# antonilo/unsupervised_detection

Measured on AMD Instinct MI355X. Metric: frame-pairs/sec per adversarial step, DAVIS 480p batch4, 1/2/4/8 GPU, higher is better.
Workload: dtype f32

## Files before the change

unsupervised_detection_amd/csrc/elementwise.h:

```cpp
#pragma once
#include "common.h"
namespace udet {
int launch_resize_bilinear_fwd(const float* x, int ldx, int x_coff, int N, int H, int W, float* y, int ldy, int y_coff,
                               int OH, int OW, int C, float mul, float div, hipStream_t s);
int launch_resize_bilinear_bwd(const float* dy, int ldy, int y_coff, int N, int OH, int OW, float* dx, int ldx, int x_coff,
                               int H, int W, int C, int accumulate, hipStream_t s);
int launch_upb_ring(const float* x, int ld, int N, int H, int W, float* xh, hipStream_t s);
int launch_upb_ring_fold(const float* dxh, int ld, int N, int H, int W, float* dx, hipStream_t s);
int launch_share_samples(float* buf, long P, int ld, int coff, int C, int copies, hipStream_t s);
int launch_fold_samples(float* buf, long P, int ld, int coff, int C, int copies, hipStream_t s);
int launch_emit_du(const float* d, const float* a, float* u, long P, int ld, int coff, int C, int act, float alpha, hipStream_t s);
int launch_pool2x2_sum(const float* du, float* dx, int N, int H, int W, int C, hipStream_t s);
int launch_pack_pwc_input(const float* i1, const float* i2, float* x8, long P, hipStream_t s);
int launch_gen_input(const float* img, const float* f, double* part, float* gin, int B, long HW, hipStream_t s);
size_t flow_stats_doubles(int B);
int launch_mask_rec_inputs(const float* logits, const float* f, float* mask, float* fin, long P, int ncalls, hipStream_t s);
int launch_pack_imgin(const float* img, float* imgin, long P, int ncalls, hipStream_t s);
int launch_losses(const float* f, const float* mask, const float* pred, long HW, int B, float cbn, float eps,
                  float num_pixels, float* part, float* losses, float* coef, float* sums, hipStream_t s);
size_t loss_part_floats(int B);
int launch_rec_loss_bwd(const float* f, const float* mask, const float* pred, float* dpred, long BHW, float cbn,
                        float inv_np, hipStream_t s);
int launch_gen_loss_bwd(const float* f, const float* mask, const float* pred, const float* coef, float* dpred,
                        float* dmask, long HW, int B, float cbn, hipStream_t s);
int launch_mask_bwd(const float* dmask, const float* dfin, const float* f, const float* mask, float* dlogits, long P,
                    hipStream_t s);
int launch_grad_absmean(const float* g, const long* seg_off, const long* seg_len, int nvars, float* vmean, float thresh,
                        float* out, hipStream_t s);
int launch_adam(float* w, float* g, float* m, float* v, long n, float lr_t, float b1, float b2, float eps, float clip,
                const float* flag, uint64_t seed, uint64_t step, hipStream_t s, int mode = 0, const int* skip = nullptr);
int launch_nonfinite_count(const float* g, long n, int* out, hipStream_t s);
int launch_flow_normalize(const float* f, double* part, float* out, int B, long HW, hipStream_t s);
int launch_charbonnier(const float* gt, const float* pred, const float* mask, int mc, int B, long HW, float cbn, float* part,
                       float* out, hipStream_t s);
int launch_crop_flip_resize(const void* src, int src_u8, int nearest, int N, int H, int W, int C, const int* prm, float* dst, int OH,
                            int OW, float div, float add, hipStream_t s);
int launch_crop_flip_resize_ragged(const void* src, int src_u8, int nearest, int N, int C, const long long* offsets, const int* hw,
                                   const int* prm, float* dst, int OH, int OW, float div, float add, hipStream_t s);
int launch_mask_stats(const float* pred, const float* gt, int N, int H, int W, float threshold, float gt_threshold, double* out,
                      hipStream_t s);
int launch_boundary_stats(const float* pred, const float* gt, const double* stats8, int N, int H, int W, float threshold,
                          float gt_threshold, int radius, unsigned long long* counts4, unsigned char* bmap_pred,
                          unsigned char* bmap_gt, hipStream_t s);
size_t restore_workspace_bytes(int n);
int launch_restore_masks_ragged(const float* masks, int n, int mh, int mw, const long long* offsets, const int* tab, const int* coef,
                                int max_h, int max_w, unsigned char* out, int* amax, unsigned char* binary, double threshold,
                                void* workspace, hipStream_t s);
size_t components_workspace_bytes(size_t total_pixels, int n);
int launch_select_components_ragged(const unsigned char* binary, const unsigned char* gt, int n, const long long* offsets, const int* hw,
                                    int max_h, int max_w, size_t total_pixels, int connectivity, int mode, int* labels,
                                    unsigned char* selected, long long* info, void* workspace, hipStream_t s);
size_t component_boxes_workspace_bytes(size_t total_pixels, int n);
int launch_component_boxes_ragged(const int* labels, const unsigned char* score, int n, const long long* offsets, const int* hw, int max_h,
                                  int max_w, size_t total_pixels, int min_area, int k, long long* dets, long long* counts, void* workspace,
                                  hipStream_t s);
int launch_draw_boxes_ragged(unsigned char* rgb, int n, const long long* offsets, const int* hw, const long long* dets,
                             const long long* counts, int k, int thickness, unsigned colour, hipStream_t s);
int launch_fill_uniform(float* x, long n, uint64_t seed, float lo, float hi, hipStream_t s);
int launch_axpy(const float* x, float* y, long n, float a, int accumulate, hipStream_t s);
}
```

unsupervised_detection_amd/csrc/elementwise.hip:

```cpp
#include "common.h"
#include "elementwise.h"

namespace udet {

static inline int grid_for(long total, int cap = 4096) {
  long nb = (total + 255) / 256;
  if (nb > cap) nb = cap;
  if (nb < 1) nb = 1;
  return (int)nb;
}

template <typename T>
__device__ __forceinline__ T wave_sum(T v) {
#pragma unroll
  for (int o = 32; o > 0; o >>= 1) v += __shfl_down(v, o, 64);
  return v;
}
template <typename T>
__device__ __forceinline__ T block_sum(T v, T* sm ) {
  v = wave_sum(v);
  __syncthreads();
  if ((threadIdx.x & 63) == 0) sm[threadIdx.x >> 6] = v;
  __syncthreads();
  return sm[0] + sm[1] + sm[2] + sm[3];
// ... 252 lines not shown
                       C / 4, accumulate);
    UDET_HIP(hipGetLastError());
    return UDET_OK;
  }
  const long total = (long)N * H * W * C;
  hipLaunchKernelGGL(resize_bilinear_bwd_kernel, dim3(grid_for(total)), dim3(256), 0, s, dy, ldy, y_coff, N, OH, OW, dx,
                     ldx, x_coff, H, W, C, accumulate);
  UDET_HIP(hipGetLastError());
  return UDET_OK;
}

__global__ __launch_bounds__(256) void pool2x2_sum_kernel(const float* __restrict__ du, float* __restrict__ dx, int N, int H,
                                                          int W, int C) {
  const int c4n = C >> 2;
  const long total = (long)N * H * W * c4n;
  for (long e = (long)blockIdx.x * 256 + threadIdx.x; e < total; e += (long)gridDim.x * 256) {
    const int c4 = (int)(e % c4n);
    const long pix = e / c4n;
    const int x = (int)(pix % W), y = (int)((pix / W) % H), n = (int)(pix / ((long)W * H));
    const float* b = du + ((((long)n * 2 * H + 2 * y) * 2 * W) + 2 * x) * C + c4 * 4;
    const float4 a0 = *reinterpret_cast<const float4*>(b), a1 = *reinterpret_cast<const float4*>(b + C);
    const float4 a2 = *reinterpret_cast<const float4*>(b + (long)2 * W * C), a3 = *reinterpret_cast<const float4*>(b + (long)2 * W * C + C);
    float4 o;
    o.x = (a0.x + a1.x) + (a2.x + a3.x);
    o.y = (a0.y + a1.y) + (a2.y + a3.y);
    o.z = (a0.z + a1.z) + (a2.z + a3.z);
    o.w = (a0.w + a1.w) + (a2.w + a3.w);
    *reinterpret_cast<float4*>(dx + pix * C + c4 * 4) = o;
  }
}
int launch_pool2x2_sum(const float* du, float* dx, int N, int H, int W, int C, hipStream_t s) {
  hipLaunchKernelGGL(pool2x2_sum_kernel, dim3(grid_for((long)N * H * W * (C / 4))), dim3(256), 0, s, du, dx, N, H, W, C);
  UDET_HIP(hipGetLastError());
  return UDET_OK;
}

__global__ __launch_bounds__(256) void emit_du_kernel(const float* __restrict__ d, const float* __restrict__ a,
                                                      float* __restrict__ u, long P, int ld, int coff, int C, int act,
                                                      float alpha) {
  const long total = P * C;
  for (long e = (long)blockIdx.x * 256 + threadIdx.x; e < total; e += (long)gridDim.x * 256) {
    const long pix = e / C;
    const long o = pix * ld + coff + (e - pix * C);
    u[o] = d[o] * act_dfo(a[o], act, alpha);
  }
}
int launch_emit_du(const float* d, const float* a, float* u, long P, int ld, int coff, int C, int act, float alpha, hipStream_t s) {
  hipLaunchKernelGGL(emit_du_kernel, dim3(grid_for(P * C)), dim3(256), 0, s, d, a, u, P, ld, coff, C, act, alpha);
  UDET_HIP(hipGetLastError());
  return UDET_OK;
}

template <int V, bool FOLD>
__global__ __launch_bounds__(256) void share_fold_kernel(float* __restrict__ buf, long P, int ld, int coff, int C, int copies) {
  const int CV = C / V;
  const long total = P * CV;
  for (long e = (long)blockIdx.x * 256 + threadIdx.x; e < total; e += (long)gridDim.x * 256) {
    const long pix = e / CV;
    const long o = pix * ld + coff + (e - pix * CV) * V;
    if (V == 4) {
      float4 v = *reinterpret_cast<const float4*>(buf + o);
      for (int k = 1; k < copies; ++k) {
        float4* q = reinterpret_cast<float4*>(buf + o + (long)k * P * ld);
        if (FOLD) {
          const float4 w = *q;
          v.x += w.x; v.y += w.y; v.z += w.z; v.w += w.w;
        } else {
          *q = v;
        }
      }
      if (FOLD) *reinterpret_cast<float4*>(buf + o) = v;
    } else {
      float v = buf[o];
      for (int k = 1; k < copies; ++k) {
        if (FOLD) v += buf[o + (long)k * P * ld];
        else buf[o + (long)k * P * ld] = v;
      }
      if (FOLD) buf[o] = v;
    }
  }
}
static int launch_share_fold(float* buf, long P, int ld, int coff, int C, int copies, bool fold, hipStream_t s) {
  if (copies < 2 || C < 1) return UDET_OK;
  const bool v4 = (ld % 4 == 0) && (coff % 4 == 0) && (C % 4 == 0);
  const long n = P * (v4 ? C / 4 : C);
  if (v4) {
    if (fold) hipLaunchKernelGGL((share_fold_kernel<4, true>), dim3(grid_for(n)), dim3(256), 0, s, buf, P, ld, coff, C, copies);
    else hipLaunchKernelGGL((share_fold_kernel<4, false>), dim3(grid_for(n)), dim3(256), 0, s, buf, P, ld, coff, C, copies);
  } else {
    if (fold) hipLaunchKernelGGL((share_fold_kernel<1, true>), dim3(grid_for(n)), dim3(256), 0, s, buf, P, ld, coff, C, copies);
    else hipLaunchKernelGGL((share_fold_kernel<1, false>), dim3(grid_for(n)), dim3(256), 0, s, buf, P, ld, coff, C, copies);
  }
  UDET_HIP(hipGetLastError());
  return UDET_OK;
}
int launch_share_samples(float* buf, long P, int ld, int coff, int C, int copies, hipStream_t s) {
  return launch_share_fold(buf, P, ld, coff, C, copies, false, s);
}
int launch_fold_samples(float* buf, long P, int ld, int coff, int C, int copies, hipStream_t s) {
  return launch_share_fold(buf, P, ld, coff, C, copies, true, s);
}

__global__ __launch_bounds__(256) void pack_pwc_input_kernel(const float* __restrict__ i1, const float* __restrict__ i2,
                                                             float* __restrict__ x8, long P) {
  for (long e = (long)blockIdx.x * 256 + threadIdx.x; e < 2 * P; e += (long)gridDim.x * 256) {
    const float* s = e < P ? i1 + e * 3 : i2 + (e - P) * 3;
    float4 a = make_float4(s[0] + 0.5f, s[1] + 0.5f, s[2] + 0.5f, 0.f);
    *reinterpret_cast<float4*>(x8 + e * 4) = a;
  }
}
int launch_pack_pwc_input(const float* i1, const float* i2, float* x8, long P, hipStream_t s) {
  hipLaunchKernelGGL(pack_pwc_input_kernel, dim3(grid_for(2 * P)), dim3(256), 0, s, i1, i2, x8, P);
  UDET_HIP(hipGetLastError());
  return UDET_OK;
}

#define FS_BLOCKS 32
__global__ __launch_bounds__(256) void flow_stats_kernel(const float* __restrict__ f, long HW, double* __restrict__ part) {
  __shared__ double sm[4];
  const int n = blockIdx.y;
  double s0 = 0, s1 = 0, q0 = 0, q1 = 0;
  for (long p = (long)blockIdx.x * 256 + threadIdx.x; p < HW; p += (long)gridDim.x * 256) {
    const float2 v = *reinterpret_cast<const float2*>(f + ((long)n * HW + p) * 2);
    s0 += v.x; s1 += v.y;
    q0 += (double)v.x * v.x; q1 += (double)v.y * v.y;
  }
  s0 = block_sum(s0, sm); s1 = block_sum(s1, sm); q0 = block_sum(q0, sm); q1 = block_sum(q1, sm);
  if (threadIdx.x == 0) {
    double* o = part + ((long)n * FS_BLOCKS + blockIdx.x) * 4;
    o[0] = s0; o[1] = s1; o[2] = q0; o[3] = q1;
  }
}
__global__ __launch_bounds__(256) void pack_gen_input_kernel(const float* __restrict__ img, const float* __restrict__ f,
                                                             const double* __restrict__ part, float* __restrict__ gin,
                                                             long HW) {
  __shared__ float st[4];
  const int n = blockIdx.y;
  if (threadIdx.x < 2) {
    double s = 0, q = 0;
    for (int b = 0; b < FS_BLOCKS; ++b) {
      s += part[((long)n * FS_BLOCKS + b) * 4 + threadIdx.x];
      q += part[((long)n * FS_BLOCKS + b) * 4 + 2 + threadIdx.x];
    }
    const double mean = s / (double)HW, var = q / (double)HW - mean * mean;
    st[threadIdx.x] = (float)mean;
    st[2 + threadIdx.x] = sqrtf((float)var);
  }
  __syncthreads();
  const float m0 = st[0], m1 = st[1], d0 = st[2], d1 = st[3];
  for (long p = (long)blockIdx.x * 256 + threadIdx.x; p < HW; p += (long)gridDim.x * 256) {
    const long q = (long)n * HW + p;
    const float2 v = *reinterpret_cast<const float2*>(f + q * 2);
    *reinterpret_cast<float4*>(gin + q * 8) = make_float4(img[q * 3], img[q * 3 + 1], img[q * 3 + 2], (v.x - m0) / d0);
// ... 60 lines not shown
  }
}
int launch_mask_rec_inputs(const float* logits, const float* f, float* mask, float* fin, long P, int ncalls, hipStream_t s) {
  hipLaunchKernelGGL(mask_rec_inputs_kernel, dim3(grid_for(P)), dim3(256), 0, s, logits, f, mask, fin, P, ncalls);
  UDET_HIP(hipGetLastError());
  return UDET_OK;
}
__global__ __launch_bounds__(256) void pack_imgin_kernel(const float* __restrict__ img, float* __restrict__ imgin, long P,
                                                         int ncalls) {
  for (long q = (long)blockIdx.x * 256 + threadIdx.x; q < P; q += (long)gridDim.x * 256) {
    const float4 im = make_float4(img[q * 3], img[q * 3 + 1], img[q * 3 + 2], 0.f);
    for (int k = 0; k < ncalls; ++k) *reinterpret_cast<float4*>(imgin + (k * P + q) * 4) = im;
  }
}
int launch_pack_imgin(const float* img, float* imgin, long P, int ncalls, hipStream_t s) {
  hipLaunchKernelGGL(pack_imgin_kernel, dim3(grid_for(P)), dim3(256), 0, s, img, imgin, P, ncalls);
  UDET_HIP(hipGetLastError());
  return UDET_OK;
}

__device__ __forceinline__ float charb(float e, float cbn) {
  const float s = e * e + 0.001f * 0.001f;
  return cbn == 0.5f ? sqrtf(s) : powf(s, cbn);
}
__device__ __forceinline__ float charb_d(float e, float cbn) {
  const float s = e * e + 0.001f * 0.001f;
  return cbn == 0.5f ? e / sqrtf(s) : cbn * powf(s, cbn - 1.f) * 2.f * e;
}
#define LS_BLOCKS 64
__global__ __launch_bounds__(256) void loss_sums_kernel(const float* __restrict__ f, const float* __restrict__ mask,
                                                        const float* __restrict__ pred , long HW, int B,
                                                        float cbn, float* __restrict__ part ) {
  __shared__ float sm[4];
  const int n = blockIdx.y;
  float R = 0, Rc = 0, Pp = 0, Dr = 0, Dc = 0;
  for (long p = (long)blockIdx.x * 256 + threadIdx.x; p < HW; p += (long)gridDim.x * 256) {
    const long q = (long)n * HW + p;
    const float2 fl = *reinterpret_cast<const float2*>(f + q * 2);
    const float2 a = *reinterpret_cast<const float2*>(pred + q * 2);
    const float2 b = *reinterpret_cast<const float2*>(pred + ((long)B * HW + q) * 2);
    const float2 c = *reinterpret_cast<const float2*>(pred + ((long)2 * B * HW + q) * 2);
    const float m = mask[q], cm = 1.f - m;
    const float pa = charb(fl.x - a.x, cbn) + charb(fl.y - a.y, cbn);
    const float pb = charb(fl.x - b.x, cbn) + charb(fl.y - b.y, cbn);
    const float pc = charb(fl.x - c.x, cbn) + charb(fl.y - c.y, cbn);
    R += pa * m; Rc += pb * cm; Pp += pc; Dr += pc * m; Dc += pc * cm;
  }
  R = block_sum(R, sm); Rc = block_sum(Rc, sm); Pp = block_sum(Pp, sm); Dr = block_sum(Dr, sm); Dc = block_sum(Dc, sm);
  if (threadIdx.x == 0) {
    float* o = part + ((long)n * LS_BLOCKS + blockIdx.x) * 5;
    o[0] = R; o[1] = Rc; o[2] = Pp; o[3] = Dr; o[4] = Dc;
  }
}
__global__ void loss_finish_kernel(const float* __restrict__ part, int B, float eps, float num_pixels,
                                   float* __restrict__ losses, float* __restrict__ coef, float* __restrict__ sums) {
  if (threadIdx.x != 0 || blockIdx.x != 0) return;
  float red = 0.f, redc = 0.f, rs = 0.f;
  for (int b = 0; b < B; ++b) {
    float v[5] = {0, 0, 0, 0, 0};
    for (int k = 0; k < LS_BLOCKS; ++k)
      for (int j = 0; j < 5; ++j) v[j] += part[((long)b * LS_BLOCKS + k) * 5 + j];
    const float D = v[3] + eps, Dc = v[4] + eps;
    red += 1.f - v[0] / D;
    redc += 1.f - v[1] / Dc;
    rs += v[0] + v[1] + v[2];
    coef[b * 4 + 0] = -1.f / (B * D);
    coef[b * 4 + 1] = v[0] / (B * D * D);
    coef[b * 4 + 2] = -1.f / (B * Dc);
    coef[b * 4 + 3] = v[1] / (B * Dc * Dc);
    for (int j = 0; j < 5; ++j) sums[b * 5 + j] = v[j];
    if (b == 0) { losses[4] = v[0]; losses[5] = v[1]; losses[6] = D; losses[7] = Dc; }
  }
  red /= B; redc /= B;
  losses[0] = red + redc;
  losses[1] = rs / num_pixels;
  losses[2] = red;
  losses[3] = redc;
}
int launch_losses(const float* f, const float* mask, const float* pred, long HW, int B, float cbn, float eps,
                  float num_pixels, float* part, float* losses, float* coef, float* sums, hipStream_t s) {
  hipLaunchKernelGGL(loss_sums_kernel, dim3(LS_BLOCKS, B), dim3(256), 0, s, f, mask, pred, HW, B, cbn, part);
  hipLaunchKernelGGL(loss_finish_kernel, dim3(1), dim3(64), 0, s, part, B, eps, num_pixels, losses, coef, sums);
  UDET_HIP(hipGetLastError());
  return UDET_OK;
}
size_t loss_part_floats(int B) { return (size_t)B * LS_BLOCKS * 5; }

__global__ __launch_bounds__(256) void charbonnier_sum_kernel(const float* __restrict__ gt, const float* __restrict__ pred,
                                                              const float* __restrict__ mask, int mc, long HW, float cbn,
                                                              float* __restrict__ part ) {
  __shared__ float sm[4];
  const int n = blockIdx.y;
  float acc = 0.f;
  for (long p = (long)blockIdx.x * 256 + threadIdx.x; p < HW; p += (long)gridDim.x * 256) {
    const long q = (long)n * HW + p;
    const float2 a = *reinterpret_cast<const float2*>(gt + q * 2);
    const float2 b = *reinterpret_cast<const float2*>(pred + q * 2);
    const float m0 = mask ? mask[q * mc] : 1.f, m1 = mask ? mask[q * mc + (mc - 1)] : 1.f;
    acc += charb(a.x - b.x, cbn) * m0 + charb(a.y - b.y, cbn) * m1;
  }
  acc = block_sum(acc, sm);
  if (threadIdx.x == 0) part[(long)n * LS_BLOCKS + blockIdx.x] = acc;
}
__global__ void charbonnier_finish_kernel(const float* __restrict__ part, int B, float* __restrict__ out) {
  const int b = blockIdx.x * blockDim.x + threadIdx.x;
  if (b >= B) return;
  float v = 0.f;
  for (int k = 0; k < LS_BLOCKS; ++k) v += part[(long)b * LS_BLOCKS + k];
  out[b] = v;
}
int launch_charbonnier(const float* gt, const float* pred, const float* mask, int mc, int B, long HW, float cbn, float* part,
                       float* out, hipStream_t s) {
  hipLaunchKernelGGL(charbonnier_sum_kernel, dim3(LS_BLOCKS, B), dim3(256), 0, s, gt, pred, mask, mc, HW, cbn, part);
  hipLaunchKernelGGL(charbonnier_finish_kernel, dim3((B + 63) / 64), dim3(64), 0, s, part, B, out);
  UDET_HIP(hipGetLastError());
  return UDET_OK;
}

__global__ __launch_bounds__(256) void rec_loss_bwd_kernel(const float* __restrict__ f, const float* __restrict__ mask,
                                                           const float* __restrict__ pred, float* __restrict__ dpred,
                                                           long BHW, float cbn, float inv_np) {
  for (long q = (long)blockIdx.x * 256 + threadIdx.x; q < BHW; q += (long)gridDim.x * 256) {
    const float2 fl = *reinterpret_cast<const float2*>(f + q * 2);
    const float m = mask[q], cm = 1.f - m;
    const float2 a = *reinterpret_cast<const float2*>(pred + q * 2);
    const float2 b = *reinterpret_cast<const float2*>(pred + (BHW + q) * 2);
    const float2 c = *reinterpret_cast<const float2*>(pred + (2 * BHW + q) * 2);
    *reinterpret_cast<float2*>(dpred + q * 2) = make_float2(-charb_d(fl.x - a.x, cbn) * m * inv_np, -charb_d(fl.y - a.y, cbn) * m * inv_np);
    *reinterpret_cast<float2*>(dpred + (BHW + q) * 2) = make_float2(-charb_d(fl.x - b.x, cbn) * cm * inv_np, -charb_d(fl.y - b.y, cbn) * cm * inv_np);
    *reinterpret_cast<float2*>(dpred + (2 * BHW + q) * 2) = make_float2(-charb_d(fl.x - c.x, cbn) * inv_np, -charb_d(fl.y - c.y, cbn) * inv_np);
  }
}
int launch_rec_loss_bwd(const float* f, const float* mask, const float* pred, float* dpred, long BHW, float cbn,
                        float inv_np, hipStream_t s) {
  hipLaunchKernelGGL(rec_loss_bwd_kernel, dim3(grid_for(BHW)), dim3(256), 0, s, f, mask, pred, dpred, BHW, cbn, inv_np);
// ... 11 lines not shown
    const float cR = coef[n * 4], cD = coef[n * 4 + 1], cRc = coef[n * 4 + 2], cDc = coef[n * 4 + 3];
    const float2 fl = *reinterpret_cast<const float2*>(f + q * 2);
    const float m = mask[q], cm = 1.f - m;
    const float2 a = *reinterpret_cast<const float2*>(pred + q * 2);
    const float2 b = *reinterpret_cast<const float2*>(pred + (BHW + q) * 2);
    const float2 c = *reinterpret_cast<const float2*>(pred + (2 * BHW + q) * 2);
    *reinterpret_cast<float2*>(dpred + q * 2) = make_float2(-cR * charb_d(fl.x - a.x, cbn) * m, -cR * charb_d(fl.y - a.y, cbn) * m);
    *reinterpret_cast<float2*>(dpred + (BHW + q) * 2) = make_float2(-cRc * charb_d(fl.x - b.x, cbn) * cm, -cRc * charb_d(fl.y - b.y, cbn) * cm);
    const float pa = charb(fl.x - a.x, cbn) + charb(fl.y - a.y, cbn);
    const float pb = charb(fl.x - b.x, cbn) + charb(fl.y - b.y, cbn);
    const float pc = charb(fl.x - c.x, cbn) + charb(fl.y - c.y, cbn);
    dmask[q] = cR * pa + cD * pc - cRc * pb - cDc * pc;
  }
}
int launch_gen_loss_bwd(const float* f, const float* mask, const float* pred, const float* coef, float* dpred,
                        float* dmask, long HW, int B, float cbn, hipStream_t s) {
  hipLaunchKernelGGL(gen_loss_bwd_kernel, dim3(grid_for((long)B * HW)), dim3(256), 0, s, f, mask, pred, coef, dpred, dmask,
                     HW, B, cbn);
  UDET_HIP(hipGetLastError());
  return UDET_OK;
}

__global__ __launch_bounds__(256) void mask_bwd_kernel(const float* __restrict__ dmask, const float* __restrict__ dfin,
                                                       const float* __restrict__ f, const float* __restrict__ mask,
                                                       float* __restrict__ dlogits , long P) {
  for (long q = (long)blockIdx.x * 256 + threadIdx.x; q < P; q += (long)gridDim.x * 256) {
    const float4 g0 = *reinterpret_cast<const float4*>(dfin + q * 4);
    const float4 g1 = *reinterpret_cast<const float4*>(dfin + (P + q) * 4);
    const float2 fl = *reinterpret_cast<const float2*>(f + q * 2);
    float dm = dmask[q];
    dm -= g0.x * fl.x + g0.y * fl.y + g0.w;
    dm += g1.x * fl.x + g1.y * fl.y + g1.w;
    const float m = mask[q];
    const float d0 = dm * m * (1.f - m) / 10.f;
    dlogits[q * 8] = d0;
    dlogits[q * 8 + 1] = -d0;
  }
}
int launch_mask_bwd(const float* dmask, const float* dfin, const float* f, const float* mask, float* dlogits, long P,
                    hipStream_t s) {
  hipLaunchKernelGGL(mask_bwd_kernel, dim3(grid_for(P)), dim3(256), 0, s, dmask, dfin, f, mask, dlogits, P);
  UDET_HIP(hipGetLastError());
  return UDET_OK;
}

#define GA_SPLIT 8
__global__ __launch_bounds__(256) void grad_absmean_kernel(const float* __restrict__ g, const long* __restrict__ seg_off,
                                                           const long* __restrict__ seg_len, float* __restrict__ vpart) {
  __shared__ float sm[4];
  const long off = seg_off[blockIdx.x], len = seg_len[blockIdx.x];
  const long b = len * blockIdx.y / GA_SPLIT, e = len * (blockIdx.y + 1) / GA_SPLIT;
  float s0 = 0.f, s1 = 0.f, s2 = 0.f, s3 = 0.f;
  long i = b + threadIdx.x;
  for (; i + 768 < e; i += 1024) {
    s0 += fabsf(g[off + i]);
    s1 += fabsf(g[off + i + 256]);
    s2 += fabsf(g[off + i + 512]);
    s3 += fabsf(g[off + i + 768]);
  }
  for (; i < e; i += 256) s0 += fabsf(g[off + i]);
  const float s = block_sum((s0 + s1) + (s2 + s3), sm);
  if (threadIdx.x == 0) vpart[blockIdx.x * GA_SPLIT + blockIdx.y] = s;
}
__global__ void grad_flag_kernel(const float* __restrict__ vpart, const long* __restrict__ seg_len, int nvars, float thresh,
                                 float* __restrict__ out ) {
  if (threadIdx.x == 0 && blockIdx.x == 0) {
    float s = 0.f;
    for (int i = 0; i < nvars; ++i) {
      float v = 0.f;
      for (int j = 0; j < GA_SPLIT; ++j) v += vpart[i * GA_SPLIT + j];
      s += v / (float)seg_len[i];
    }
    s /= (float)nvars;
    out[0] = s;
    out[1] = s < thresh ? 1.f : 0.f;
  }
}
int launch_grad_absmean(const float* g, const long* seg_off, const long* seg_len, int nvars, float* vmean, float thresh,
                        float* out, hipStream_t s) {
  hipLaunchKernelGGL(grad_absmean_kernel, dim3(nvars, GA_SPLIT), dim3(256), 0, s, g, seg_off, seg_len, vmean);
  hipLaunchKernelGGL(grad_flag_kernel, dim3(1), dim3(64), 0, s, vmean, seg_len, nvars, thresh, out);
  UDET_HIP(hipGetLastError());
  return UDET_OK;
}

__device__ __host__ __forceinline__ float udet_uniform01(uint64_t seed, uint64_t step, uint64_t idx) {
  uint64_t z = seed * 0x9E3779B97F4A7C15ull + step * 0xBF58476D1CE4E5B9ull + idx + 0x94D049BB133111EBull;
  z = (z ^ (z >> 30)) * 0xBF58476D1CE4E5B9ull;
  z = (z ^ (z >> 27)) * 0x94D049BB133111EBull;
  z = z ^ (z >> 31);
  return (float)(z >> 40) * (1.0f / 16777216.0f);
}

__global__ __launch_bounds__(256) void adam_kernel(float* __restrict__ w, float* __restrict__ g, float* __restrict__ m,
                                                   float* __restrict__ v, long n, float lr_t, float b1, float b2, float eps,
                                                   float clip, const float* __restrict__ flag, uint64_t seed,
                                                   uint64_t step, int mode, const int* __restrict__ skip) {
  if (skip && *skip != 0) return;
  const bool noise = flag && flag[1] != 0.f;
  for (long i = (long)blockIdx.x * 256 + threadIdx.x; i < n; i += (long)gridDim.x * 256) {
    float gi = g[i];
    if (mode != 2) {
      if (noise) gi = fabsf((udet_uniform01(seed, step, (uint64_t)i) * 2.f - 1.f) * clip);
      else gi = fminf(fmaxf(gi, -clip), clip);
      g[i] = gi;
      if (mode == 1) continue;
    }
    const float mi = m[i] + (gi - m[i]) * (1.f - b1);
    const float vi = v[i] + (gi * gi - v[i]) * (1.f - b2);
    m[i] = mi;
    v[i] = vi;
    w[i] = w[i] - lr_t * mi / (sqrtf(vi) + eps);
  }
}
__global__ __launch_bounds__(256) void fill_uniform_kernel(float* __restrict__ x, long n, uint64_t seed, float lo, float hi) {
  for (long i = (long)blockIdx.x * 256 + threadIdx.x; i < n; i += (long)gridDim.x * 256)
    x[i] = lo + (hi - lo) * udet_uniform01(seed, 0, (uint64_t)i);
}
int launch_fill_uniform(float* x, long n, uint64_t seed, float lo, float hi, hipStream_t s) {
  hipLaunchKernelGGL(fill_uniform_kernel, dim3(grid_for(n, 8192)), dim3(256), 0, s, x, n, seed, lo, hi);
  UDET_HIP(hipGetLastError());
  return UDET_OK;
}
__global__ __launch_bounds__(256) void mask_stats_kernel(const float* __restrict__ pred, const float* __restrict__ gt, int H, int W,
                                                         float threshold, float gt_threshold, double* __restrict__ out) {
  __shared__ double sm[4];
  const int n = blockIdx.x;
  const long HW = (long)H * W;
  double v[8] = {0, 0, 0, 0, 0, 0, 0, 0};
  for (long q = threadIdx.x; q < HW; q += 256) {
    const int y = (int)(q / W), x = (int)(q - (long)y * W);
    const float g = gt[n * HW + q];
    const bool pr = pred[n * HW + q] > threshold, gb = g > gt_threshold;
    const int strips = (y < 2) + (y >= H - 2) + (x < 2) + (x >= W - 2);
// ... 116 lines not shown
```

unsupervised_detection_amd/csrc/plan_step.hip:

```cpp
#include "conv_host.h"
#include "elementwise.h"
#include "plan_run.h"

namespace udet {

static const int PWC_CH[7] = {0, 16, 32, 64, 96, 128, 196};
static const char* const WARP_NAME[7] = {"", "", "warp_costvol2", "warp_costvol3", "warp_costvol4", "warp_costvol5", "warp_costvol6"};

static int pwc_forward_on(Plan* P, const float* img1, const float* img2, float* ws, const Lane& L0, const Lane& LH) {
  if (!P->pwc_packed) {
    set_error("pwc_forward: call udet_pack_pwc first");
    return UDET_ERR_ARG;
  }
  const Config& c = P->cfg;
  const Resolved& R = P->R;
  const int B = c.batch;
  hipStream_t s = L0.s;
  auto fwd = [&](int layer, int N, const Lane& ln) { return run_fwd(P, P->pwc[layer], N, ws, ln); };
  UDET_TRY(launch_pack_pwc_input(img1, img2, ws + P->buf(R.pwc_x8).off, (long)B * c.in_h * c.in_w, s));
  for (int l = 1; l <= 6; ++l)
    for (int j = 0; j < 3; ++j) UDET_TRY(fwd(R.pwc.pyr[l][j], 2 * B, L0));
  for (int l = 6; l >= 2; --l) {
    const int h = c.in_h >> l, w = c.in_w >> l, C = PWC_CH[l];
    const Buf& cb = P->buf(R.pwc_c[l]);
// ... 25 lines not shown
  if (P->prefetch_pending) (void)hipStreamWaitEvent(s, P->prefetch_ev, 0);
  return pwc_forward_on(P, img1, img2, ws, lane_of(P, s, 0), lane_of(P, s, 2));
}

static int plan_prepare_image(Plan* P, const float* img1, int dst, float* ws, hipStream_t s) {
  const Config& c = P->cfg;
  return launch_resize_bilinear_fwd(img1, 3, 0, c.batch, c.in_h, c.in_w, ws + P->buf(dst).off, 3, 0, c.img_h, c.img_w,
                                    3, 1.f, 1.f, s);
}
static int plan_prepare_flow(Plan* P, int dst, float* ws, hipStream_t s) {
  const Config& c = P->cfg;
  const Buf& ff = P->buf(P->R.flow_full);
  return launch_resize_bilinear_fwd(ws + ff.off, 2, 0, c.batch, c.in_h, c.in_w, ws + P->buf(dst).off, 2, 0, c.img_h,
                                    c.img_w, 2, 1.f, c.flow_normalizer, s);
}

int plan_prefetch(Plan* P, const float* img1, const float* img2, float* ws, hipStream_t s) {
  const Lane L0 = lane_of(P, s, 0), LC = lane_of(P, s, 4), LH = lane_of(P, s, 5);
  P->in_prefetch = true;
  P->ev_next_prefetch = 0;
  order_after(P, L0, LC);
  int rc = pwc_forward_on(P, img1, img2, ws, LC, LH);
  P->in_prefetch = false;
  UDET_TRY(rc);
  UDET_TRY(plan_prepare_flow(P, P->R.flow_next, ws, LC.s));
  UDET_TRY(plan_prepare_image(P, img1, P->R.image_next, ws, LC.s));
  if (!P->prefetch_ev) (void)hipEventCreateWithFlags(&P->prefetch_ev, hipEventDisableTiming);
  (void)hipEventRecord(P->prefetch_ev, LC.s);
  P->prefetch_pending = true;
  return UDET_OK;
}

int plan_generator_forward(Plan* P, float* ws, hipStream_t s) {
  const Config& c = P->cfg;
  const long HW = (long)c.img_h * c.img_w;
  const Lane L0 = lane_of(P, s, 0);
  double* part = reinterpret_cast<double*>(ws + P->small_off + 4096);
  UDET_TRY(launch_gen_input(ws + P->buf(P->R.image).off, ws + P->buf(P->R.flow).off, part, ws + P->buf(P->R.gen_in).off, c.batch, HW, s));
  for (const auto& L : P->gen) UDET_TRY(run_fwd(P, L, c.batch, ws, L0));
  return UDET_OK;
}
int plan_generator_layers(Plan* P, float* ws, hipStream_t s) {
  const Lane L0 = lane_of(P, s, 0);
  for (const auto& L : P->gen) UDET_TRY(run_fwd(P, L, P->cfg.batch, ws, L0));
  return UDET_OK;
}

static int rec_resize(Plan* P, int src, int dst, int N, float* ws, hipStream_t s) {
  const Buf &a = P->buf(src), &b = P->buf(dst);
  return launch_resize_bilinear_fwd(ws + a.off, a.ld, 0, N, a.h, a.w, ws + b.off, b.ld, 0, b.h, b.w, a.ld, 1.f, 1.f, s);
}
static int dec_src(const Resolved& R, int k) { return k == 5 ? R.rec_conv6 : R.rec_concat[k + 1]; }

static int share_enc_a_output(Plan* P, const Layer& L, int ncalls, float* ws, hipStream_t s) {
  const Buf& y = P->buf(L.y);
  if (ncalls > 1 && L.y_fanned_out) return launch_share_samples(ws + y.off, (long)P->cfg.batch * y.h * y.w, y.ld, L.y_coff, L.cout, ncalls, s);
  return UDET_OK;
}
static int plan_rec_image_branch(Plan* P, int ncalls, float* ws, const Lane& ln, bool with_layers = true) {
  const Config& c = P->cfg;
  if (ncalls < 1) return UDET_OK;
  const long Ppix = (long)c.batch * c.img_h * c.img_w;
  UDET_TRY(launch_pack_imgin(ws + P->buf(P->R.image).off, ws + P->buf(P->R.rec_imgin).off, Ppix, 1, ln.s));
  if (!with_layers) return UDET_OK;
  for (int i = 0; i < 9; ++i) {
    const Layer& L = P->rec[P->R.rec.enc[0][i]];
    UDET_TRY(run_fwd(P, L, c.batch, ws, ln));
    UDET_TRY(share_enc_a_output(P, L, ncalls, ws, ln.s));
  }
  P->enc_a_shared = true;
  return UDET_OK;
}

int plan_recover_forward(Plan* P, int ncalls, float* ws, hipStream_t s, bool inputs_prepacked, bool skip_enc_a, bool enc_a_input_packed) {
  const Config& c = P->cfg;
  const Resolved& R = P->R;
  const int B = c.batch, N = ncalls * B;
  const long Ppix = (long)B * c.img_h * c.img_w;
  const Lane L0 = lane_of(P, s, 0);
  if (!inputs_prepacked)
    UDET_TRY(launch_mask_rec_inputs(ws + P->buf(R.gen_a17).off, ws + P->buf(R.flow).off, ws + P->buf(R.mask).off, ws + P->buf(R.rec_fin).off,
                                    Ppix, ncalls, s));
  if (ncalls < 1) return UDET_OK;
  auto enc = [&](int e, int i) -> const Layer& { return P->rec[R.rec.enc[e][i]]; };
  if (!skip_enc_a && pairs_on(P)) {
    if (!inputs_prepacked && !enc_a_input_packed) UDET_TRY(plan_rec_image_branch(P, ncalls, ws, L0, false));
    for (int i = 0; i < 9; ++i) {
      const Layer& La = enc(0, i);
      UDET_TRY(run_fwd_pair(P, La, inputs_prepacked ? N : B, enc(1, i), N, ws, L0));
      if (!inputs_prepacked) UDET_TRY(share_enc_a_output(P, La, ncalls, ws, s));
    }
    P->enc_a_shared = !inputs_prepacked;
  } else {
    if (!skip_enc_a) {
      if (inputs_prepacked) {
        for (int i = 0; i < 9; ++i) UDET_TRY(run_fwd(P, enc(0, i), N, ws, L0));
        P->enc_a_shared = false;
      } else {
        UDET_TRY(plan_rec_image_branch(P, ncalls, ws, L0));
      }
    }
    for (int i = 0; i < 9; ++i) UDET_TRY(run_fwd(P, enc(1, i), N, ws, L0));
  }
  for (int k = 5; k >= 1; --k) {
    const Layer& dcl = P->rec[R.rec.deconv[k]];
    if (!dcl.upb) UDET_TRY(rec_resize(P, dec_src(R, k), R.rec_r[k + 1], N, ws, s));
    UDET_TRY(run_fwd(P, dcl, N, ws, L0));
    if (k < 5) {
      UDET_TRY(rec_resize(P, R.rec_flow[k + 1], R.rec_rf[k + 1], N, ws, s));
      UDET_TRY(run_fwd(P, P->rec[R.rec.upflow[k]], N, ws, L0));
    }
    UDET_TRY(run_fwd(P, P->rec[R.rec.flow[k]], N, ws, L0));
  }
  const Buf& f1 = P->buf(R.rec_flow[1]);
  return launch_resize_bilinear_fwd(ws + f1.off, f1.ld, 0, N, f1.h, f1.w, ws + P->buf(R.pred).off, 2, 0, c.img_h, c.img_w, 2, 1.f, 1.f, s);
}

int plan_losses(Plan* P, float* ws, hipStream_t s) {
  const Config& c = P->cfg;
  float* sm = ws + P->small_off;
  const long HW = (long)c.img_h * c.img_w;
  return launch_losses(ws + P->buf(P->R.flow).off, ws + P->buf(P->R.mask).off, ws + P->buf(P->R.pred).off, HW,
                       c.batch, c.cbn, c.epsilon, (float)(c.img_w * c.img_h * c.batch), sm + 8192, sm, sm + 16, sm + UDET_SMALL_SUMS, s);
}

int plan_prefetch_consume(Plan* P, float* ws, hipStream_t s) {
  if (!P->prefetch_pending) {
    set_error("forward_prefetched: no udet_prefetch_flow is pending");
    return UDET_ERR_ARG;
  }
  (void)hipStreamWaitEvent(s, P->prefetch_ev, 0);
  P->prefetch_pending = false;
  const Buf &fn = P->buf(P->R.flow_next), &in = P->buf(P->R.image_next);
  UDET_HIP(hipMemcpyAsync(ws + P->buf(P->R.flow).off, ws + fn.off, fn.floats() * sizeof(float), hipMemcpyDeviceToDevice, s));
  UDET_HIP(hipMemcpyAsync(ws + P->buf(P->R.image).off, ws + in.off, in.floats() * sizeof(float), hipMemcpyDeviceToDevice, s));
  return UDET_OK;
}

int plan_forward(Plan* P, const float* img1, const float* img2, int ncalls, float* ws, hipStream_t s, bool prefetched) {
  P->ev_next = 0;
  const Lane L0 = lane_of(P, s, 0), LI = lane_of(P, s, 1);
  if (prefetched) {
    UDET_TRY(plan_prefetch_consume(P, ws, s));
    img1 = img2 = nullptr;
// ... 32 lines not shown
    return run_wgrad(P, L, n < 0 ? N : n, dy, is_du, w_rec, g_rec, ws, lw);
  };
  auto wgrad = [&](const Layer& L, int dy, bool is_du, int n = -1) -> int { return wgrad_on(LW, L, dy, is_du, n); };
  auto wgrad_dec = [&](const Layer& L, int dy, bool is_du) -> int { return wgrad_on(LWdec, L, dy, is_du, -1); };
  const Lane LA = LAp ? *LAp : LD;
  const bool a_own_lane = LA.s != LD.s;
  const int ncopies = N / c.batch;
  const bool a_shared = P->enc_a_shared && ncopies > 1;
  const Emit none;
  const float LEAK = 0.2f;
  {
    const Buf& df1 = P->buf(G.flow[1]);
    UDET_TRY(launch_resize_bilinear_bwd(ws + P->buf(G.pred).off, 2, 0, N, c.img_h, c.img_w, ws + df1.off, df1.ld, 0, df1.h, df1.w, 2, 0, s));
  }
  for (int k = 1; k <= 5; ++k) {
    const int dconcat = G.concat[k], uconcat = G.u_concat[k];
    const Layer* fl = &P->rec[R.rec.flow[k]];
    const Layer* dc = &P->rec[R.rec.deconv[k]];
    Emit em;
    em.ubuf = uconcat; em.abuf = fl->x; em.c0 = 0; em.c1 = dc->cout; em.act = ACT_LEAKY; em.alpha = LEAK;
    UDET_TRY(run_dgrad(P, *fl, N, G.flow[k], false, dconcat, 0, k == 1 ? 0 : 1, -1, em, ws, LD));
    if (with_wgrad) UDET_TRY(wgrad_dec(*fl, G.flow[k], false));
    if (k < 5) {
      const Layer* uf = &P->rec[R.rec.upflow[k]];
      if (with_wgrad) UDET_TRY(wgrad_dec(*uf, dconcat, false));
      UDET_TRY(run_dgrad(P, *uf, N, dconcat, false, G.rf[k + 1], 0, 0, -1, none, ws, LD));
      const Buf &drf = P->buf(G.rf[k + 1]), &dfn = P->buf(G.flow[k + 1]);
      UDET_TRY(launch_resize_bilinear_bwd(ws + drf.off, drf.ld, 0, N, drf.h, drf.w, ws + dfn.off, dfn.ld, 0, dfn.h, dfn.w, drf.ld, 0, s));
    }
    if (with_wgrad) {
      if (dc->upb) {
        order_after(P, LD, LWdec);
        UDET_TRY(rec_resize(P, dec_src(R, k), R.rec_r[k + 1], N, ws, LWdec.s));
      }
      UDET_TRY(wgrad_dec(*dc, uconcat, true));
    }
    if (dc->upb_bwd) {
      UDET_TRY(run_dgrad_upb(P, *dc, N, uconcat, G.p[k + 1], G.concat[k + 1], ws, LD));
      continue;
    }
    const int dr = G.r[k + 1];
    UDET_TRY(run_dgrad(P, *dc, N, uconcat, true, dr, 0, 0, -1, none, ws, LD));
    const Buf& bdr = P->buf(dr);
    const Buf& dsrc = P->buf(k == 5 ? G.conv6 : G.concat[k + 1]);
    UDET_TRY(launch_resize_bilinear_bwd(ws + bdr.off, bdr.ld, 0, N, bdr.h, bdr.w, ws + dsrc.off, dsrc.ld, 0, dsrc.h, dsrc.w,
                                        bdr.ld, 0, s));
  }
  {
    const Buf &d6 = P->buf(G.conv6), &a6 = P->buf(R.rec_conv6), &u6 = P->buf(G.u_conv6);
    UDET_TRY(launch_emit_du(ws + d6.off, ws + a6.off, ws + u6.off, (long)N * d6.h * d6.w, d6.ld, 0, d6.ld, ACT_LEAKY, LEAK, s));
  }
  if (a_own_lane) order_after(P, LD, LA);
  const bool pair_enc = pairs_on(P, 1) && with_wgrad && !a_own_lane;
  for (int i = 8; i >= 0; --i) {
    DgradJob job[2];
    int njob = 0;
    for (int e = 0; e < 2; ++e) {
      if (e == 0 && !with_wgrad) continue;
      const Layer* L = &P->rec[R.rec.enc[e][i]];
      const int du = G.enc_du[e][i];
      const bool shared = e == 0 && a_shared;
      const int Ne = shared ? c.batch : N;
      const bool own = e == 0 && a_own_lane;
      const Lane& LE = own ? LA : LD;
      hipStream_t se = LE.s;
      if (shared && i == 8) {
        const Buf& u = P->buf(du);
        UDET_TRY(launch_fold_samples(ws + u.off, (long)c.batch * u.h * u.w, u.ld, L->y_coff, L->cout, ncopies, se));
      }
      if (with_wgrad) {
        if (own) UDET_TRY(run_wgrad(P, *L, Ne, du, true, w_rec, g_rec, ws, LA));
        else UDET_TRY(wgrad(*L, du, true, Ne));
      }
      if (i == 0) {
        if (e == 1 && need_dfin) UDET_TRY(run_dgrad(P, *L, N, du, true, G.fin, 0, 0, -1, none, ws, LD));
        continue;
      }
      const int dx = G.enc_dx[e][i];
      const bool slab_in = L->x_in_slab;
      Emit em;
      em.ubuf = G.enc_ux[e][i]; em.abuf = L->x; em.c0 = 0; em.c1 = L->cin; em.act = ACT_LEAKY; em.alpha = LEAK;
      if (shared && slab_in) {
        const Buf& d = P->buf(dx);
        UDET_TRY(launch_fold_samples(ws + d.off, (long)c.batch * d.h * d.w, d.ld, L->x_coff, L->cin, ncopies, se));
      }
      if (pair_enc) {
        job[njob].L = L; job[njob].N = Ne; job[njob].dy = du; job[njob].dx = dx; job[njob].dx_coff = L->x_coff;
        job[njob].accumulate = slab_in ? 1 : 0; job[njob].em = em;
        ++njob;
        continue;
      }
      UDET_TRY(run_dgrad(P, *L, Ne, du, true, dx, L->x_coff, slab_in ? 1 : 0, -1, em, ws, LE));
    }
    if (njob == 2) UDET_TRY(run_dgrad_pair(P, job[0], job[1], ws, LD));
    else if (njob == 1) UDET_TRY(run_dgrad(P, *job[0].L, job[0].N, job[0].dy, true, job[0].dx, job[0].dx_coff, job[0].accumulate, -1, job[0].em, ws, LD));
  }
  if (a_own_lane) order_after(P, LA, LD);
  if (with_wgrad && LWdec.s != LW.s) order_after(P, LWdec, LD);
  return UDET_OK;
}

static int backward_recover(Plan* P, const float* w_rec, float* g_rec, float* ws, const Lane& LD, const Lane& LW, const Lane* LA = nullptr,
                            const Lane* LWdec = nullptr) {
  const Config& c = P->cfg;
  const Resolved& R = P->R;
  const long BHW = (long)c.batch * c.img_h * c.img_w;
  UDET_TRY(launch_rec_loss_bwd(ws + P->buf(R.flow).off, ws + P->buf(R.mask).off, ws + P->buf(R.pred).off, ws + P->buf(R.grad[0].pred).off, BHW,
                               c.cbn, 1.0f / (float)(c.img_w * c.img_h * c.batch), LD.s));
  return rec_backward(P, 3 * c.batch, R.grad[0], true, false, w_rec, g_rec, ws, LD, LW, LA, LWdec);
}

static int backward_generator(Plan* P, const float* w_gen, float* g_gen, float* ws, const Lane& LD, const Lane& LW, const Lane* LWlate = nullptr,
                              int nlate = 0) {
  const Config& c = P->cfg;
  const Resolved& R = P->R;
  const int B = c.batch;
  const long HW = (long)c.img_h * c.img_w;
  hipStream_t s = LD.s;
  float* sm = ws + P->small_off;
  UDET_TRY(launch_gen_loss_bwd(ws + P->buf(R.flow).off, ws + P->buf(R.mask).off, ws + P->buf(R.pred).off, sm + 16,
                               ws + P->buf(R.grad[1].pred).off, ws + P->buf(R.d_mask).off, HW, B, c.cbn, s));
  UDET_TRY(rec_backward(P, 2 * B, R.grad[1], false, true, nullptr, nullptr, ws, LD, LD));
  UDET_TRY(launch_mask_bwd(ws + P->buf(R.d_mask).off, ws + P->buf(R.grad[1].fin).off, ws + P->buf(R.flow).off, ws + P->buf(R.mask).off,
                           ws + P->buf(R.gen_d[17]).off, B * HW, s));
  for (int i = 16; i >= 0; --i) {
    const Layer& L = P->gen[i];
    const bool has_act = L.act != ACT_NONE;
    const int dy = has_act ? R.gen_u[i + 1] : R.gen_d[i + 1];
    const Lane& LWi = (LWlate && i < nlate) ? *LWlate : LW;
    order_after(P, LD, LWi);
    UDET_TRY(run_wgrad(P, L, B, dy, has_act, w_gen, g_gen, ws, LWi));
    if (i == 0) break;
    const int res = i == 6 ? R.gen_d[11] : (i == 3 ? R.gen_d[14] : (i == 1 ? R.gen_d[15] : -1));
    const int dx = R.gen_d[i];
    const Layer& Lp = P->gen[i - 1];
    const int ap = Lp.y2 >= 0 ? Lp.y2 : Lp.y;
    {
      Emit em;
// ... 46 lines not shown
```

Baseline: 501.7.

## Batch share/fold sample kernels into segmented launches and parallelize reduction finishers

The per-layer share and fold kernels for the shared encoder-A branch are collected into one segmented kernel launch, taking up to 8 buffers at a time. The segment table is passed by value, and each block finds its segment from a prefix table of block offsets. This replaces many small launches in forward and backward. In backward, all folds are now issued up front on the A lane instead of interleaved with the dgrad loop, which changes stream ordering and relies on the decoder contributions already being present in those buffers. Separately, the single-thread loss-finish and grad-flag kernels now read their partial sums in parallel across 256 threads, and the grad abs-mean loop is unrolled to issue more loads at once.

Result: no change. 502.4 (median of 6 runs) (+0.2%).

```diff
diff --git a/unsupervised_detection_amd/csrc/elementwise.h b/unsupervised_detection_amd/csrc/elementwise.h
--- a/unsupervised_detection_amd/csrc/elementwise.h
+++ b/unsupervised_detection_amd/csrc/elementwise.h
@@ -7,8 +7,14 @@
                                int H, int W, int C, int accumulate, hipStream_t s);
 int launch_upb_ring(const float* x, int ld, int N, int H, int W, float* xh, hipStream_t s);
 int launch_upb_ring_fold(const float* dxh, int ld, int N, int H, int W, float* dx, hipStream_t s);
-int launch_share_samples(float* buf, long P, int ld, int coff, int C, int copies, hipStream_t s);
-int launch_fold_samples(float* buf, long P, int ld, int coff, int C, int copies, hipStream_t s);
+#define SHARE_MAX_SEGS 8
+struct ShareSeg {
+  float* buf;
+  long P;
+  int ld, coff, C;
+};
+int launch_share_samples_segs(const ShareSeg* seg, int nseg, int copies, hipStream_t s);
+int launch_fold_samples_segs(const ShareSeg* seg, int nseg, int copies, hipStream_t s);
 int launch_emit_du(const float* d, const float* a, float* u, long P, int ld, int coff, int C, int act, float alpha, hipStream_t s);
 int launch_pool2x2_sum(const float* du, float* dx, int N, int H, int W, int C, hipStream_t s);
 int launch_pack_pwc_input(const float* i1, const float* i2, float* x8, long P, hipStream_t s);
diff --git a/unsupervised_detection_amd/csrc/elementwise.hip b/unsupervised_detection_amd/csrc/elementwise.hip
--- a/unsupervised_detection_amd/csrc/elementwise.hip
+++ b/unsupervised_detection_amd/csrc/elementwise.hip
@@ -328,10 +328,10 @@
 }
 
 template <int V, bool FOLD>
-__global__ __launch_bounds__(256) void share_fold_kernel(float* __restrict__ buf, long P, int ld, int coff, int C, int copies) {
+__device__ __forceinline__ void share_fold_segment(float* __restrict__ buf, long P, int ld, int coff, int C, int copies, int bx, int nbx) {
   const int CV = C / V;
   const long total = P * CV;
-  for (long e = (long)blockIdx.x * 256 + threadIdx.x; e < total; e += (long)gridDim.x * 256) {
+  for (long e = (long)bx * 256 + threadIdx.x; e < total; e += (long)nbx * 256) {
     const long pix = e / CV;
     const long o = pix * ld + coff + (e - pix * CV) * V;
     if (V == 4) {
@@ -356,6 +356,53 @@
     }
   }
 }
+template <int V, bool FOLD>
+__global__ __launch_bounds__(256) void share_fold_kernel(float* __restrict__ buf, long P, int ld, int coff, int C, int copies) {
+  share_fold_segment<V, FOLD>(buf, P, ld, coff, C, copies, blockIdx.x, gridDim.x);
+}
+struct ShareSegs {
+  ShareSeg s[SHARE_MAX_SEGS];
+  int blk0[SHARE_MAX_SEGS + 1];
+  int n;
+};
+template <bool FOLD>
+__global__ __launch_bounds__(256) void share_fold_segs_kernel(ShareSegs segs, int copies) {
+  int k = 0;
+  while (k + 1 < segs.n && (int)blockIdx.x >= segs.blk0[k + 1]) ++k;
+  const ShareSeg& sg = segs.s[k];
+  share_fold_segment<4, FOLD>(sg.buf, sg.P, sg.ld, sg.coff, sg.C, copies, (int)blockIdx.x - segs.blk0[k], segs.blk0[k + 1] - segs.blk0[k]);
+}
+static int launch_share_fold(float* buf, long P, int ld, int coff, int C, int copies, bool fold, hipStream_t s);
+static int launch_share_fold_segs(const ShareSeg* seg, int nseg, int copies, bool fold, hipStream_t s) {
+  if (copies < 2) return UDET_OK;
+  ShareSegs a;
+  a.n = 0;
+  a.blk0[0] = 0;
+  auto flush = [&]() -> int {
+    if (a.n == 1) UDET_TRY(launch_share_fold(a.s[0].buf, a.s[0].P, a.s[0].ld, a.s[0].coff, a.s[0].C, copies, fold, s));
+    if (a.n > 1) {
+      if (fold) hipLaunchKernelGGL((share_fold_segs_kernel<true>), dim3(a.blk0[a.n]), dim3(256), 0, s, a, copies);
+      else hipLaunchKernelGGL((share_fold_segs_kernel<false>), dim3(a.blk0[a.n]), dim3(256), 0, s, a, copies);
+      UDET_HIP(hipGetLastError());
+    }
+    a.n = 0;
+    return UDET_OK;
+  };
+  for (int i = 0; i < nseg; ++i) {
+    const ShareSeg& g = seg[i];
+    if (g.C < 1 || g.P < 1) continue;
+    if ((g.ld % 4) || (g.coff % 4) || (g.C % 4)) {
+      UDET_TRY(launch_share_fold(g.buf, g.P, g.ld, g.coff, g.C, copies, fold, s));
+      continue;
+    }
+    a.s[a.n] = g;
+    a.blk0[a.n + 1] = a.blk0[a.n] + grid_for(g.P * (g.C / 4));
+    if (++a.n == SHARE_MAX_SEGS) UDET_TRY(flush());
+  }
+  return flush();
+}
+int launch_share_samples_segs(const ShareSeg* seg, int nseg, int copies, hipStream_t s) { return launch_share_fold_segs(seg, nseg, copies, false, s); }
+int launch_fold_samples_segs(const ShareSeg* seg, int nseg, int copies, hipStream_t s) { return launch_share_fold_segs(seg, nseg, copies, true, s); }
 static int launch_share_fold(float* buf, long P, int ld, int coff, int C, int copies, bool fold, hipStream_t s) {
   if (copies < 2 || C < 1) return UDET_OK;
   const bool v4 = (ld % 4 == 0) && (coff % 4 == 0) && (C % 4 == 0);
@@ -369,12 +416,6 @@
   }
   UDET_HIP(hipGetLastError());
   return UDET_OK;
-}
-int launch_share_samples(float* buf, long P, int ld, int coff, int C, int copies, hipStream_t s) {
-  return launch_share_fold(buf, P, ld, coff, C, copies, false, s);
-}
-int launch_fold_samples(float* buf, long P, int ld, int coff, int C, int copies, hipStream_t s) {
-  return launch_share_fold(buf, P, ld, coff, C, copies, true, s);
 }
 
 __global__ __launch_bounds__(256) void pack_pwc_input_kernel(const float* __restrict__ i1, const float* __restrict__ i2,
@@ -541,25 +582,50 @@
     o[0] = R; o[1] = Rc; o[2] = Pp; o[3] = Dr; o[4] = Dc;
   }
 }
-__global__ void loss_finish_kernel(const float* __restrict__ part, int B, float eps, float num_pixels,
-                                   float* __restrict__ losses, float* __restrict__ coef, float* __restrict__ sums) {
-  if (threadIdx.x != 0 || blockIdx.x != 0) return;
+#define LF_THREADS 256
+#define LF_SAMPLES 51
+#define LF_BATCH 16
+__global__ __launch_bounds__(LF_THREADS) void loss_finish_kernel(const float* __restrict__ part, int B, float eps, float num_pixels,
+                                                                 float* __restrict__ losses, float* __restrict__ coef,
+                                                                 float* __restrict__ sums) {
+  __shared__ float sv[LF_SAMPLES * 5];
+  if (blockIdx.x != 0) return;
   float red = 0.f, redc = 0.f, rs = 0.f;
-  for (int b = 0; b < B; ++b) {
-    float v[5] = {0, 0, 0, 0, 0};
-    for (int k = 0; k < LS_BLOCKS; ++k)
-      for (int j = 0; j < 5; ++j) v[j] += part[((long)b * LS_BLOCKS + k) * 5 + j];
-    const float D = v[3] + eps, Dc = v[4] + eps;
-    red += 1.f - v[0] / D;
-    redc += 1.f - v[1] / Dc;
-    rs += v[0] + v[1] + v[2];
-    coef[b * 4 + 0] = -1.f / (B * D);
-    coef[b * 4 + 1] = v[0] / (B * D * D);
-    coef[b * 4 + 2] = -1.f / (B * Dc);
-    coef[b * 4 + 3] = v[1] / (B * Dc * Dc);
-    for (int j = 0; j < 5; ++j) sums[b * 5 + j] = v[j];
-    if (b == 0) { losses[4] = v[0]; losses[5] = v[1]; losses[6] = D; losses[7] = Dc; }
-  }
+  for (int b0 = 0; b0 < B; b0 += LF_SAMPLES) {
+    const int nb = B - b0 < LF_SAMPLES ? B - b0 : LF_SAMPLES;
+    if ((int)threadIdx.x < nb * 5) {
+      const int b = b0 + (int)threadIdx.x / 5, j = (int)threadIdx.x % 5;
+      const float* p = part + (long)b * LS_BLOCKS * 5 + j;
+      float v = 0.f;
+      for (int k0 = 0; k0 < LS_BLOCKS; k0 += LF_BATCH) {
+        float t[LF_BATCH];
+#pragma unroll
+        for (int k = 0; k < LF_BATCH; ++k) t[k] = p[(k0 + k) * 5];
+#pragma unroll
+        for (int k = 0; k < LF_BATCH; ++k) v += t[k];
+      }
+      sv[threadIdx.x] = v;
+    }
+    __syncthreads();
+    if (threadIdx.x == 0) {
+      for (int b = b0; b < b0 + nb; ++b) {
+        float v[5];
+        for (int j = 0; j < 5; ++j) v[j] = sv[(b - b0) * 5 + j];
+        const float D = v[3] + eps, Dc = v[4] + eps;
+        red += 1.f - v[0] / D;
+        redc += 1.f - v[1] / Dc;
+        rs += v[0] + v[1] + v[2];
+        coef[b * 4 + 0] = -1.f / (B * D);
+        coef[b * 4 + 1] = v[0] / (B * D * D);
+        coef[b * 4 + 2] = -1.f / (B * Dc);
+        coef[b * 4 + 3] = v[1] / (B * Dc * Dc);
+        for (int j = 0; j < 5; ++j) sums[b * 5 + j] = v[j];
+        if (b == 0) { losses[4] = v[0]; losses[5] = v[1]; losses[6] = D; losses[7] = Dc; }
+      }
+    }
+    __syncthreads();
+  }
+  if (threadIdx.x != 0) return;
   red /= B; redc /= B;
   losses[0] = red + redc;
   losses[1] = rs / num_pixels;
@@ -569,7 +635,7 @@
 int launch_losses(const float* f, const float* mask, const float* pred, long HW, int B, float cbn, float eps,
                   float num_pixels, float* part, float* losses, float* coef, float* sums, hipStream_t s) {
   hipLaunchKernelGGL(loss_sums_kernel, dim3(LS_BLOCKS, B), dim3(256), 0, s, f, mask, pred, HW, B, cbn, part);
-  hipLaunchKernelGGL(loss_finish_kernel, dim3(1), dim3(64), 0, s, part, B, eps, num_pixels, losses, coef, sums);
+  hipLaunchKernelGGL(loss_finish_kernel, dim3(1), dim3(LF_THREADS), 0, s, part, B, eps, num_pixels, losses, coef, sums);
   UDET_HIP(hipGetLastError());
   return UDET_OK;
 }
@@ -687,6 +753,20 @@
   const long b = len * blockIdx.y / GA_SPLIT, e = len * (blockIdx.y + 1) / GA_SPLIT;
   float s0 = 0.f, s1 = 0.f, s2 = 0.f, s3 = 0.f;
   long i = b + threadIdx.x;
+  for (; i + 768 + 3 * 1024 < e; i += 4 * 1024) {
+    float t[4][4];
+#pragma unroll
+    for (int m = 0; m < 4; ++m)
+#pragma unroll
+      for (int j = 0; j < 4; ++j) t[m][j] = g[off + i + m * 1024 + j * 256];
+#pragma unroll
+    for (int m = 0; m < 4; ++m) {
+      s0 += fabsf(t[m][0]);
+      s1 += fabsf(t[m][1]);
+      s2 += fabsf(t[m][2]);
+      s3 += fabsf(t[m][3]);
+    }
+  }
   for (; i + 768 < e; i += 1024) {
     s0 += fabsf(g[off + i]);
     s1 += fabsf(g[off + i + 256]);
@@ -697,24 +777,38 @@
   const float s = block_sum((s0 + s1) + (s2 + s3), sm);
   if (threadIdx.x == 0) vpart[blockIdx.x * GA_SPLIT + blockIdx.y] = s;
 }
-__global__ void grad_flag_kernel(const float* __restrict__ vpart, const long* __restrict__ seg_len, int nvars, float thresh,
-                                 float* __restrict__ out ) {
-  if (threadIdx.x == 0 && blockIdx.x == 0) {
-    float s = 0.f;
-    for (int i = 0; i < nvars; ++i) {
+#define GF_THREADS 256
+__global__ __launch_bounds__(GF_THREADS) void grad_flag_kernel(const float* __restrict__ vpart, const long* __restrict__ seg_len, int nvars,
+                                                               float thresh, float* __restrict__ out ) {
+  __shared__ float sq[GF_THREADS];
+  if (blockIdx.x != 0) return;
+  float s = 0.f;
+  for (int i0 = 0; i0 < nvars; i0 += GF_THREADS) {
+    const int n = nvars - i0 < GF_THREADS ? nvars - i0 : GF_THREADS;
+    if ((int)threadIdx.x < n) {
+      const int i = i0 + (int)threadIdx.x;
+      float t[GA_SPLIT];
+#pragma unroll
+      for (int j = 0; j < GA_SPLIT; ++j) t[j] = vpart[i * GA_SPLIT + j];
       float v = 0.f;
-      for (int j = 0; j < GA_SPLIT; ++j) v += vpart[i * GA_SPLIT + j];
-      s += v / (float)seg_len[i];
-    }
-    s /= (float)nvars;
-    out[0] = s;
-    out[1] = s < thresh ? 1.f : 0.f;
-  }
+#pragma unroll
+      for (int j = 0; j < GA_SPLIT; ++j) v += t[j];
+      sq[threadIdx.x] = v / (float)seg_len[i];
+    }
+    __syncthreads();
+    if (threadIdx.x == 0)
+      for (int i = 0; i < n; ++i) s += sq[i];
+    __syncthreads();
+  }
+  if (threadIdx.x != 0) return;
+  s /= (float)nvars;
+  out[0] = s;
+  out[1] = s < thresh ? 1.f : 0.f;
 }
 int launch_grad_absmean(const float* g, const long* seg_off, const long* seg_len, int nvars, float* vmean, float thresh,
                         float* out, hipStream_t s) {
   hipLaunchKernelGGL(grad_absmean_kernel, dim3(nvars, GA_SPLIT), dim3(256), 0, s, g, seg_off, seg_len, vmean);
-  hipLaunchKernelGGL(grad_flag_kernel, dim3(1), dim3(64), 0, s, vmean, seg_len, nvars, thresh, out);
+  hipLaunchKernelGGL(grad_flag_kernel, dim3(1), dim3(GF_THREADS), 0, s, vmean, seg_len, nvars, thresh, out);
   UDET_HIP(hipGetLastError());
   return UDET_OK;
 }
diff --git a/unsupervised_detection_amd/csrc/plan_step.hip b/unsupervised_detection_amd/csrc/plan_step.hip
--- a/unsupervised_detection_amd/csrc/plan_step.hip
+++ b/unsupervised_detection_amd/csrc/plan_step.hip
@@ -101,10 +101,17 @@
 }
 static int dec_src(const Resolved& R, int k) { return k == 5 ? R.rec_conv6 : R.rec_concat[k + 1]; }
 
-static int share_enc_a_output(Plan* P, const Layer& L, int ncalls, float* ws, hipStream_t s) {
-  const Buf& y = P->buf(L.y);
-  if (ncalls > 1 && L.y_fanned_out) return launch_share_samples(ws + y.off, (long)P->cfg.batch * y.h * y.w, y.ld, L.y_coff, L.cout, ncalls, s);
-  return UDET_OK;
+static int share_enc_a_outputs(Plan* P, int ncalls, float* ws, hipStream_t s) {
+  if (ncalls < 2) return UDET_OK;
+  ShareSeg seg[9];
+  int n = 0;
+  for (int i = 0; i < 9; ++i) {
+    const Layer& L = P->rec[P->R.rec.enc[0][i]];
+    if (!L.y_fanned_out) continue;
+    const Buf& y = P->buf(L.y);
+    seg[n++] = ShareSeg{ws + y.off, (long)P->cfg.batch * y.h * y.w, y.ld, L.y_coff, L.cout};
+  }
+  return launch_share_samples_segs(seg, n, ncalls, s);
 }
 static int plan_rec_image_branch(Plan* P, int ncalls, float* ws, const Lane& ln, bool with_layers = true) {
   const Config& c = P->cfg;
@@ -112,11 +119,8 @@
   const long Ppix = (long)c.batch * c.img_h * c.img_w;
   UDET_TRY(launch_pack_imgin(ws + P->buf(P->R.image).off, ws + P->buf(P->R.rec_imgin).off, Ppix, 1, ln.s));
   if (!with_layers) return UDET_OK;
-  for (int i = 0; i < 9; ++i) {
-    const Layer& L = P->rec[P->R.rec.enc[0][i]];
-    UDET_TRY(run_fwd(P, L, c.batch, ws, ln));
-    UDET_TRY(share_enc_a_output(P, L, ncalls, ws, ln.s));
-  }
+  for (int i = 0; i < 9; ++i) UDET_TRY(run_fwd(P, P->rec[P->R.rec.enc[0][i]], c.batch, ws, ln));
+  UDET_TRY(share_enc_a_outputs(P, ncalls, ws, ln.s));
   P->enc_a_shared = true;
   return UDET_OK;
 }
@@ -134,11 +138,8 @@
   auto enc = [&](int e, int i) -> const Layer& { return P->rec[R.rec.enc[e][i]]; };
   if (!skip_enc_a && pairs_on(P)) {
     if (!inputs_prepacked && !enc_a_input_packed) UDET_TRY(plan_rec_image_branch(P, ncalls, ws, L0, false));
-    for (int i = 0; i < 9; ++i) {
-      const Layer& La = enc(0, i);
-      UDET_TRY(run_fwd_pair(P, La, inputs_prepacked ? N : B, enc(1, i), N, ws, L0));
-      if (!inputs_prepacked) UDET_TRY(share_enc_a_output(P, La, ncalls, ws, s));
-    }
+    for (int i = 0; i < 9; ++i) UDET_TRY(run_fwd_pair(P, enc(0, i), inputs_prepacked ? N : B, enc(1, i), N, ws, L0));
+    if (!inputs_prepacked) UDET_TRY(share_enc_a_outputs(P, ncalls, ws, s));
     P->enc_a_shared = !inputs_prepacked;
   } else {
     if (!skip_enc_a) {
@@ -277,6 +278,22 @@
   }
   if (a_own_lane) order_after(P, LD, LA);
   const bool pair_enc = pairs_on(P, 1) && with_wgrad && !a_own_lane;
+  if (a_shared && with_wgrad) {
+    ShareSeg seg[9];
+    int n = 0;
+    for (int i = 8; i >= 1; --i) {
+      const Layer& L = P->rec[R.rec.enc[0][i]];
+      if (i == 8) {
+        const Buf& u = P->buf(G.enc_du[0][i]);
+        seg[n++] = ShareSeg{ws + u.off, (long)c.batch * u.h * u.w, u.ld, L.y_coff, L.cout};
+      }
+      if (L.x_in_slab) {
+        const Buf& d = P->buf(G.enc_dx[0][i]);
+        seg[n++] = ShareSeg{ws + d.off, (long)c.batch * d.h * d.w, d.ld, L.x_coff, L.cin};
+      }
+    }
+    UDET_TRY(launch_fold_samples_segs(seg, n, ncopies, LA.s));
+  }
   for (int i = 8; i >= 0; --i) {
     DgradJob job[2];
     int njob = 0;
@@ -288,11 +305,6 @@
       const int Ne = shared ? c.batch : N;
       const bool own = e == 0 && a_own_lane;
       const Lane& LE = own ? LA : LD;
-      hipStream_t se = LE.s;
-      if (shared && i == 8) {
-        const Buf& u = P->buf(du);
-        UDET_TRY(launch_fold_samples(ws + u.off, (long)c.batch * u.h * u.w, u.ld, L->y_coff, L->cout, ncopies, se));
-      }
       if (with_wgrad) {
         if (own) UDET_TRY(run_wgrad(P, *L, Ne, du, true, w_rec, g_rec, ws, LA));
         else UDET_TRY(wgrad(*L, du, true, Ne));
@@ -305,10 +317,6 @@
       const bool slab_in = L->x_in_slab;
       Emit em;
       em.ubuf = G.enc_ux[e][i]; em.abuf = L->x; em.c0 = 0; em.c1 = L->cin; em.act = ACT_LEAKY; em.alpha = LEAK;
-      if (shared && slab_in) {
-        const Buf& d = P->buf(dx);
-        UDET_TRY(launch_fold_samples(ws + d.off, (long)c.batch * d.h * d.w, d.ld, L->x_coff, L->cin, ncopies, se));
-      }
       if (pair_enc) {
         job[njob].L = L; job[njob].N = Ne; job[njob].dy = du; job[njob].dx = dx; job[njob].dx_coff = L->x_coff;
         job[njob].accumulate = slab_in ? 1 : 0; job[njob].em = em;
```
